# aa2il/pySDR

Hardware: AMD Instinct MI355X
Metric: complex IQ MS/s through 4-RX demod chain (higher is better)
Workload: dtype f32; 1 GPU; C3: 8 MS/s synthetic IQ, 4 RX (USB/CW/NFM/AM), 255-tap prototype 3/500, + 64k-FFT RF PSD on every sample; 2048 chunks x 170666 in HBM; parallelism=stream-sharded x1

## Files before the change

### pysdr_amd/csrc/api.hip

```cpp
#include <dlfcn.h>
#include <rccl/rccl.h>
#include <rocfft/rocfft.h>

#include <cmath>
#include <algorithm>
#include <cstdarg>
#include <map>

#include "common.h"
#include "host_plan.h"
#include "host_res.h"
#include "mixdec_mfma_geom.h"
#include "mixdec_plan.h"
#include "objects_plan.h"

namespace pysdr {

static thread_local char g_err[2048] = "";

void set_last_error(const char* fmt, ...) {
  va_list ap;
  va_start(ap, fmt);
  vsnprintf(g_err, sizeof(g_err), fmt, ap);
  va_end(ap);
// ... 1262 lines not shown
    float pk = 0.f;
    rc = pysdr_fetch(c, r, outs[r].am, outs[r].iq, outs[r].cap, &nout, &cx, nullptr, &pk);
    if (rc) return rc;
    outs[r].n_out = nout;
    outs[r].am_is_complex = cx;
    outs[r].peak_in = pk;
  }
  return PYSDR_OK;
}

int pysdr_quad_mixer(int device, const float* x, float* y, size_t n, uint32_t phase0,
                     uint32_t fword, uint32_t* phase_out) {
  if (!x || !y) return PYSDR_ERR_ARG;
  int rc = use_device(device);
  if (rc) return rc;
  if (phase_out) *phase_out = phase0 + fword * (uint32_t)n;
  if (n == 0) return PYSDR_OK;
  DevBuf<float2> dx, dy;
  PYSDR_HIP_CHECK(dx.alloc(n));
  PYSDR_HIP_CHECK(dy.alloc(n));
  PYSDR_HIP_CHECK(hipMemcpy(dx.get(), x, n * sizeof(float2), hipMemcpyHostToDevice));
  rc = launch_quad_mixer(dx.get(), dy.get(), n, phase0, fword, nullptr);
  if (rc) return rc;
  PYSDR_HIP_CHECK(hipMemcpy(y, dy.get(), n * sizeof(float2), hipMemcpyDeviceToHost));
  return PYSDR_OK;
}

int pysdr_fir_real(int device, const float* xx, const float* h, int ntaps, float* y, size_t n) {
  if (!xx || !h || !y || ntaps < 1) return PYSDR_ERR_ARG;
  if (n == 0) return PYSDR_OK;
  int rc = use_device(device);
  if (rc) return rc;
  const size_t nin = n + (size_t)ntaps - 1;
  DevBuf<float> dx, dh, dy;
  PYSDR_HIP_CHECK(dx.alloc(nin));
  PYSDR_HIP_CHECK(dh.alloc((size_t)ntaps));
  PYSDR_HIP_CHECK(dy.alloc(n));
  PYSDR_HIP_CHECK(hipMemcpy(dx.get(), xx, nin * sizeof(float), hipMemcpyHostToDevice));
  PYSDR_HIP_CHECK(hipMemcpy(dh.get(), h, (size_t)ntaps * sizeof(float), hipMemcpyHostToDevice));
  rc = launch_fir_real(dx.get(), dh.get(), ntaps, dy.get(), (int)n, nullptr);
  if (rc) return rc;
  PYSDR_HIP_CHECK(hipMemcpy(y, dy.get(), n * sizeof(float), hipMemcpyDeviceToHost));
  return PYSDR_OK;
}

static int get_plan(pysdr_spectrum* sp, int batch, rocfft_plan* out) {
  auto it = sp->plans.find(batch);
  if (it != sp->plans.end()) { *out = it->second; return PYSDR_OK; }
  rocfft_plan plan = nullptr;
  size_t len[1] = {(size_t)sp->nfft};
  rocfft_status s = rocfft_plan_create(&plan, rocfft_placement_inplace, rocfft_transform_type_complex_forward,
                                       rocfft_precision_single, 1, len, (size_t)batch, nullptr);
  if (s != rocfft_status_success) { set_last_error("rocfft_plan_create(nfft=%d,batch=%d) = %d", sp->nfft, batch, (int)s); return PYSDR_ERR_FFT; }
  size_t wbs = 0;
  rocfft_plan_get_work_buffer_size(plan, &wbs);
  const hipError_t e = sp->d_fftwork.grow(wbs);
  if (e != hipSuccess) {
    rocfft_plan_destroy(plan);
    set_last_error("rocFFT work buffer of %zu bytes: %s", wbs, hipGetErrorString(e));
    return PYSDR_ERR_HIP;
  }
  if (sp->d_fftwork) rocfft_execution_info_set_work_buffer(sp->info, sp->d_fftwork.get(), sp->d_fftwork.size());
  sp->plans[batch] = plan;
  *out = plan;
  return PYSDR_OK;
}

static int spectrum_alloc(pysdr_spectrum* sp, const float* window) {
  PYSDR_HIP_CHECK(sp->stream.create(hipStreamNonBlocking));
  PYSDR_HIP_CHECK(sp->d_win.alloc((size_t)sp->chunk));
  PYSDR_HIP_CHECK(hipMemcpy(sp->d_win.get(), window, (size_t)sp->chunk * sizeof(float), hipMemcpyHostToDevice));
  PYSDR_HIP_CHECK(sp->d_in.alloc((size_t)sp->chunk));
  PYSDR_HIP_CHECK(sp->d_out.alloc((size_t)sp->nfft));
  PYSDR_HIP_CHECK(sp->ev[0].create());
  PYSDR_HIP_CHECK(sp->ev[1].create());
  return PYSDR_OK;
}

int pysdr_spectrum_create(int device, int chunk_size, int nfft, int max_frames, const float* window,
                          pysdr_spectrum** out) {
  if (!out || !window || chunk_size < 1 || nfft < chunk_size || max_frames < 1) return PYSDR_ERR_ARG;
  int rc = use_device(device);
  if (rc) return rc;
  {
    std::lock_guard<std::mutex> lk(g_rocfft_mu);
    if (g_rocfft_users++ == 0) rocfft_setup();
  }
  pysdr_spectrum* sp = new pysdr_spectrum();
  sp->device = device; sp->chunk = chunk_size; sp->nfft = nfft; sp->max_frames = max_frames;
  sp->tune = SpectrumTuning::from_env();
  {
    hipDeviceProp_t prop;
    if (hipGetDeviceProperties(&prop, device) == hipSuccess && prop.multiProcessorCount > 0) sp->num_cus = prop.multiProcessorCount;
  }
  rc = spectrum_alloc(sp, window);
  if (rc) { failed_in("pysdr_spectrum_create", rc); pysdr_spectrum_destroy(sp); return rc; }
  if (rocfft_execution_info_create(&sp->info) != rocfft_status_success ||
      rocfft_execution_info_set_stream(sp->info, sp->stream.get()) != rocfft_status_success) {
    set_last_error("rocfft_execution_info_create failed");
    pysdr_spectrum_destroy(sp);
    return PYSDR_ERR_FFT;
  }
  *out = sp;
  return PYSDR_OK;
}

void pysdr_spectrum_destroy(pysdr_spectrum* sp) {
  if (!sp) return;
  (void)hipSetDevice(sp->device);
  if (sp->stream) (void)hipStreamSynchronize(sp->stream);
  for (int i = 1; i < pysdr_spectrum::kMaxStreams; ++i) if (sp->xstream[i]) (void)hipStreamSynchronize(sp->xstream[i]);
  for (auto& kv : sp->plans) rocfft_plan_destroy(kv.second);
  if (sp->info) rocfft_execution_info_destroy(sp->info);
  delete sp;
  std::lock_guard<std::mutex> lk(g_rocfft_mu);
  if (--g_rocfft_users == 0) rocfft_cleanup();
}

static int ensure_work(pysdr_spectrum* sp, size_t frames) {
  const size_t n = frames * (size_t)sp->nfft;
  if (sp->d_work.size() >= n) return PYSDR_OK;
  PYSDR_HIP_CHECK(hipStreamSynchronize(sp->stream));
  PYSDR_HIP_CHECK(sp->d_work.grow(n));
  return PYSDR_OK;
}

static int spectrum_run(pysdr_spectrum* sp, const float2* d_x, size_t hop, int nframes, int is_complex,
                        int db, float* d_out) {
  int rc;
  if (is_complex && sp->chunk == 32768 && sp->nfft == 65536 && !sp->tune.force_rocfft) {
    const int group = sp->tune.frames_per_group();
    if (sp->tune.nstreams > 1 && nframes > group) {
      const int ns = sp->tune.nstreams;
      const int part = (group + ns - 1) / ns;
      rc = ensure_work(sp, (size_t)part);
      if (rc) return rc;
      if (sp->xwork_frames < (size_t)part) {
        for (int i = 1; i < ns; ++i) {
          if (!sp->xstream[i]) PYSDR_HIP_CHECK(sp->xstream[i].create(hipStreamNonBlocking));
          if (!sp->ev_join[i]) PYSDR_HIP_CHECK(sp->ev_join[i].create(hipEventDisableTiming));
          PYSDR_HIP_CHECK(hipStreamSynchronize(sp->xstream[i]));
          PYSDR_HIP_CHECK(sp->xwork[i].alloc((size_t)part * sp->nfft));
        }
        sp->xwork_frames = (size_t)part;
      }
      PYSDR_HIP_CHECK(hipEventRecord(sp->ev[0], sp->stream));
      for (int i = 1; i < ns; ++i) PYSDR_HIP_CHECK(hipStreamWaitEvent(sp->xstream[i], sp->ev[0], 0));
      int k = 0;
      for (int f0 = 0; f0 < nframes; f0 += part, ++k) {
        const int nf = (nframes - f0 < part) ? nframes - f0 : part;
        const int w = k % ns;
        rc = launch_psd64k(d_x + (size_t)f0 * hop, hop, nf, sp->d_win.get(), w ? sp->xwork[w].get() : sp->d_work.get(),
                           d_out + (size_t)f0 * sp->nfft, db, w ? sp->xstream[w].get() : sp->stream.get(),
                           psd_form(sp->tune, nf, sp->num_cus));
        if (rc) break;
      }
      for (int i = 1; i < ns; ++i) {
        PYSDR_HIP_CHECK(hipEventRecord(sp->ev_join[i], sp->xstream[i]));
        PYSDR_HIP_CHECK(hipStreamWaitEvent(sp->stream, sp->ev_join[i], 0));
      }
      PYSDR_HIP_CHECK(hipEventRecord(sp->ev[1], sp->stream));
      return rc;
    }
    rc = ensure_work(sp, (size_t)std::min(group, nframes));
    if (rc) return rc;
    PYSDR_HIP_CHECK(hipEventRecord(sp->ev[0], sp->stream));
    for (int f0 = 0; f0 < nframes; f0 += group) {
      const int nf = (nframes - f0 < group) ? nframes - f0 : group;
      rc = launch_psd64k(d_x + (size_t)f0 * hop, hop, nf, sp->d_win.get(), sp->d_work.get(),
                         d_out + (size_t)f0 * sp->nfft, db, sp->stream, psd_form(sp->tune, nf, sp->num_cus));
      if (rc) return rc;
    }
    PYSDR_HIP_CHECK(hipEventRecord(sp->ev[1], sp->stream));
    return PYSDR_OK;
  }
  rocfft_plan plan;
  rc = get_plan(sp, nframes, &plan);
  if (rc) return rc;
  rc = ensure_work(sp, (size_t)nframes);
  if (rc) return rc;
  PYSDR_HIP_CHECK(hipEventRecord(sp->ev[0], sp->stream));
  rc = launch_psd_pre(d_x, hop, nframes, sp->chunk, sp->nfft, sp->d_win.get(), sp->d_work.get(), is_complex, sp->stream);
  if (rc) return rc;
  void* bufs[1] = {sp->d_work.get()};
  rocfft_status s = rocfft_execute(plan, bufs, nullptr, sp->info);
  if (s != rocfft_status_success) { set_last_error("rocfft_execute = %d", (int)s); return PYSDR_ERR_FFT; }
  rc = launch_psd_post(sp->d_work.get(), nframes, sp->nfft, is_complex ? 0 : 1, db, d_out, sp->stream);
  if (rc) return rc;
  PYSDR_HIP_CHECK(hipEventRecord(sp->ev[1], sp->stream));
  return PYSDR_OK;
}

int pysdr_spectrum_frame(pysdr_spectrum* sp, const float* x, int is_complex, int db, float* psd_out,
                         int* n_out) {
  if (!sp || !x || !psd_out) return PYSDR_ERR_ARG;
  int rc = use_device(sp->device);
  if (rc) return rc;
  const size_t bytes = (size_t)sp->chunk * (is_complex ? sizeof(float2) : sizeof(float));
  PYSDR_HIP_CHECK(hipMemcpyAsync(sp->d_in.get(), x, bytes, hipMemcpyHostToDevice, sp->stream));
  rc = spectrum_run(sp, sp->d_in.get(), 0, 1, is_complex, db, sp->d_out.get());
  if (!rc) sp->ran = true;
  if (rc) return rc;
  const int nout = is_complex ? sp->nfft : sp->nfft / 2;
  PYSDR_HIP_CHECK(hipMemcpyAsync(psd_out, sp->d_out.get(), (size_t)nout * sizeof(float), hipMemcpyDeviceToHost, sp->stream));
  PYSDR_HIP_CHECK(hipStreamSynchronize(sp->stream));
  if (n_out) *n_out = nout;
  return PYSDR_OK;
}

int pysdr_spectrum_batch(pysdr_spectrum* sp, const void* d_iq, int nframes, size_t hop, void* d_out) {
  if (!sp || !d_iq || !d_out || nframes < 1 || nframes > sp->max_frames) return PYSDR_ERR_ARG;
  int rc = use_device(sp->device);
  if (rc) return rc;
  rc = spectrum_run(sp, reinterpret_cast<const float2*>(d_iq), hop, nframes, 1, 1, reinterpret_cast<float*>(d_out));
  if (!rc) sp->ran = true;
  return rc;
}

int pysdr_spectrum_get_tuning(pysdr_spectrum* sp, int32_t out[4]) {
  if (!sp || !out) return PYSDR_ERR_ARG;
  out[0] = sp->tune.frames_per_group(); out[1] = sp->tune.force_rocfft ? 1 : 0; out[2] = sp->tune.nstreams; out[3] = sp->tune.packed;
  return PYSDR_OK;
}

int pysdr_spectrum_sync(pysdr_spectrum* sp) {
  if (!sp) return PYSDR_ERR_ARG;
  int rc = use_device(sp->device);
  if (rc) return rc;
  PYSDR_HIP_CHECK(hipStreamSynchronize(sp->stream));
  return PYSDR_OK;
}

int pysdr_spectrum_elapsed_ms(pysdr_spectrum* sp, float* ms) {
  if (!sp || !ms) return PYSDR_ERR_ARG;
  int rc = use_device(sp->device);
  if (rc) return rc;
  PYSDR_HIP_CHECK(hipEventSynchronize(sp->ev[1]));
  PYSDR_HIP_CHECK(hipEventElapsedTime(ms, sp->ev[0], sp->ev[1]));
  return PYSDR_OK;
}

int pysdr_spectrum_order(pysdr_spectrum* sp, pysdr_ctx* c, int direction) {
  if (!sp || !c || direction < 0 || direction > 2 || sp->device != c->cfg.device) return PYSDR_ERR_ARG;
  std::lock_guard<std::recursive_mutex> run_lk(c->run_mu);
  int rc = use_device(sp->device);
  if (rc) return rc;
  if (direction == 2) {
    c->front_wanted = 1;
    if (c->front_marker) {
      PYSDR_HIP_CHECK(hipStreamWaitEvent(sp->stream, c->front_marker, 0));
      return PYSDR_OK;
    }
    direction = 0;
  }
  if (direction == 1 && sp->ran) {
    PYSDR_HIP_CHECK(hipStreamWaitEvent(c->stream, sp->ev[1], 0));
    return PYSDR_OK;
  }
  if (!sp->ev_order) PYSDR_HIP_CHECK(sp->ev_order.create(hipEventDisableTiming));
  if (direction == 0) { rc = flush_tail(c); if (rc) return rc; }
  hipStream_t first = direction == 0 ? c->stream : sp->stream;
  hipStream_t then = direction == 0 ? sp->stream : c->stream;
  PYSDR_HIP_CHECK(hipEventRecord(sp->ev_order, first));
  PYSDR_HIP_CHECK(hipStreamWaitEvent(then, sp->ev_order, 0));
  return PYSDR_OK;
}

int pysdr_dev_alloc(int device, size_t bytes, void** out) {
  if (!out || bytes == 0) return PYSDR_ERR_ARG;
  int rc = use_device(device);
  if (rc) return rc;
  PYSDR_HIP_CHECK(hipMalloc(out, bytes));
  return PYSDR_OK;
}
int pysdr_dev_free(int device, void* p) {
  if (!p) return PYSDR_OK;
  int rc = use_device(device);
  if (rc) return rc;
  PYSDR_HIP_CHECK(hipFree(p));
  return PYSDR_OK;
}
int pysdr_dev_upload(int device, void* dst, const void* src_host, size_t bytes) {
  if (!dst || !src_host) return PYSDR_ERR_ARG;
  int rc = use_device(device);
  if (rc) return rc;
  PYSDR_HIP_CHECK(hipMemcpy(dst, src_host, bytes, hipMemcpyHostToDevice));
  return PYSDR_OK;
}
int pysdr_dev_download(int device, void* dst_host, const void* src, size_t bytes) {
  if (!dst_host || !src) return PYSDR_ERR_ARG;
  int rc = use_device(device);
  if (rc) return rc;
  PYSDR_HIP_CHECK(hipMemcpy(dst_host, src, bytes, hipMemcpyDeviceToHost));
  return PYSDR_OK;
}
int pysdr_dev_copy(int device, void* dst, const void* src, size_t bytes) {
  if (!dst || !src) return PYSDR_ERR_ARG;
  int rc = use_device(device);
  if (rc) return rc;
  PYSDR_HIP_CHECK(hipMemcpy(dst, src, bytes, hipMemcpyDeviceToDevice));
  return PYSDR_OK;
}

void pysdr_ingest_destroy(pysdr_ingest* g) {
  if (!g) return;
  if (g->c) (void)hipSetDevice(g->c->cfg.device);
  if (g->copy_stream) (void)hipStreamSynchronize(g->copy_stream);
  if (g->c && g->c->stream) (void)hipStreamSynchronize(g->c->stream);
  if (g->c && g->counted) { g->c->n_ingest--; g->counted = false; }
  delete g;
}

static int ingest_alloc(pysdr_ingest* g) {
  const int nslots = g->nslots;
  PYSDR_HIP_CHECK(g->copy_stream.create(hipStreamNonBlocking));
  g->h_in.resize(nslots);
  g->ev_copied.resize(nslots);
  g->ev_done.resize(nslots);
  g->h_am.resize((size_t)nslots * PYSDR_MAX_RX);
  g->h_iq.resize((size_t)nslots * PYSDR_MAX_RX);
  g->h_peak.resize(nslots);
  g->n_out.assign(nslots, 0);
  g->in_flight.assign(nslots, 0);
// ... 217 lines not shown
```

### pysdr_amd/csrc/host_plan.h

```cpp
#pragma once

#include <algorithm>
#include <cmath>
#include <cstdlib>
#include <cstring>

#include "common.h"

namespace pysdr {

constexpr double kTwo32 = 4294967296.0;
constexpr double kPllBwHz = 50.0, kPllZeta = 0.7071;
constexpr double kWfmPllBwHz = 30.0;
constexpr int kPllSegMax = 8192;

inline const char* tuning_env(const char* name) {
  const char* on = getenv("PYSDR_TUNING");
  if (!on || atoi(on) <= 0) return nullptr;
  return getenv(name);
}

struct Tuning {
  int tile_bytes = 0, threads = 1024;
  int wgs_per_cu = 1;
  int grid_override = 0;
  int resamp_plain = 0;
  int mfma_enable = 1;
  int dbg_flags = 0, yflush_cap = 0;
  int overlap_env = -1;
  int tail_first = -1;
  bool overlap_prio_set = false;
  int overlap_prio = 0;
  double am_taus = 16.0, am_taus_exact = 5.0;
  int am_coarse_sweeps = 4, am_kmax = 2048, am_tmin = 512;
  int am_seeded = 1, am_wseed = 0;
  int am_direct = 1;
  int am_phase_on_2 = 1;
  double wfm_taus = 20.0, wfm_taus_fast = 13.0, wfm_taus_exact = 4.0;
  int wfm_coarse_sweeps = 3, wfm_kmax = 1536, wfm_tmin = 2048;
  double wfm_taus_hi = 0.0, wfm_taus_mid = 0.0;
  int wfm_tail_cap = 0;
  int wfm_exact_cap = 5;
  int wfm_seeded = 1, wfm_wseed = 0;

  static Tuning from_env() {
    Tuning t;
    { const char* e = tuning_env("PYSDR_MIXDEC_WGS"); if (e && atoi(e) > 0) t.wgs_per_cu = atoi(e); }
    { const char* e = tuning_env("PYSDR_MIXDEC_YFLUSH"); if (e && atoi(e) > 0) t.yflush_cap = atoi(e); }
    { const char* e = tuning_env("PYSDR_AM_PLL");
      if (e && *e) {
        double a = 0, tx = 0; int cs = 0, km = 0, tm = 0;
        const int nf = sscanf(e, "%lf,%lf,%d,%d,%d", &a, &tx, &cs, &km, &tm);
        if (nf >= 1 && a > 0) t.am_taus = a;
        if (nf >= 2 && tx >= 0) t.am_taus_exact = tx;
        if (nf >= 3 && cs >= 0) t.am_coarse_sweeps = std::min(cs, 8);
        if (nf >= 4 && km > 0) t.am_kmax = std::min(km, kPllSegMax);
        if (nf >= 5 && tm >= 64) t.am_tmin = (tm + 63) & ~63;
      } }
    { const char* e = tuning_env("PYSDR_AM_SEED");
      if (e && *e) { int on = 1, ws = 0; const int nf = sscanf(e, "%d,%d", &on, &ws); if (nf >= 1) t.am_seeded = on ? 1 : 0; if (nf >= 2 && ws >= 0) t.am_wseed = ws; } }
    { const char* e = tuning_env("PYSDR_AM_DIRECT"); if (e && *e) t.am_direct = atoi(e) ? 1 : 0; }
    { const char* e = tuning_env("PYSDR_AM_PHASE_STREAM"); if (e && *e) t.am_phase_on_2 = atoi(e) ? 1 : 0; }
    { const char* e = tuning_env("PYSDR_MIXDEC_MFMA"); if (e && *e) t.mfma_enable = atoi(e) ? 1 : 0; }
    { const char* e = tuning_env("PYSDR_WFM_SEED");
      if (e && *e) { int on = 1, ws = 0; const int nf = sscanf(e, "%d,%d", &on, &ws); if (nf >= 1) t.wfm_seeded = on ? 1 : 0; if (nf >= 2 && ws >= 0) t.wfm_wseed = ws; } }
    { const char* e = tuning_env("PYSDR_OVERLAP_ORDER"); if (e && *e) t.tail_first = atoi(e); }
    { const char* e = tuning_env("PYSDR_OVERLAP"); if (e && *e) t.overlap_env = std::max(0, std::min(2, atoi(e))); }
    { const char* e = tuning_env("PYSDR_OVERLAP_PRIO"); if (e && *e) { t.overlap_prio_set = true; t.overlap_prio = atoi(e); } }
    { const char* e = tuning_env("PYSDR_RESAMP_PLAIN"); if (e && *e) t.resamp_plain = atoi(e); }
    { const char* e = tuning_env("PYSDR_MIXDEC_GRID"); if (e && atoi(e) > 0) t.grid_override = atoi(e); }
    { const char* e = tuning_env("PYSDR_WFM_PLL");
      if (e && *e) {
        double a = t.wfm_taus, b = t.wfm_taus_fast, x = t.wfm_taus_exact;
        int sw = t.wfm_coarse_sweeps, km = t.wfm_kmax, tm = t.wfm_tmin, xc = t.wfm_exact_cap;
        double th = t.wfm_taus_hi, tmid = t.wfm_taus_mid;
        int tc = t.wfm_tail_cap;
        const int got = sscanf(e, "%lf,%lf,%lf,%d,%d,%d,%d,%lf,%lf,%d", &a, &b, &x, &sw, &km, &tm, &xc, &th, &tmid, &tc);
        if (got >= 10 && tc >= 0) t.wfm_tail_cap = tc;
        if (got >= 9 && th >= 0 && tmid >= 0) { t.wfm_taus_hi = th; t.wfm_taus_mid = tmid; }
        if (got >= 7 && xc >= 0) t.wfm_exact_cap = xc;
        if (got >= 1 && a > 0) t.wfm_taus = a;
        if (got >= 2 && b >= 0) t.wfm_taus_fast = b;
        if (got >= 3 && x > 0) t.wfm_taus_exact = x;
        if (got >= 4 && sw >= 0) t.wfm_coarse_sweeps = sw;
        if (got >= 5 && km >= 1) t.wfm_kmax = std::min(km, kPllSegMax);
        if (got >= 6 && tm >= 64) t.wfm_tmin = tm;
      } }
#ifdef PYSDR_DIAG
    { const char* e = getenv("PYSDR_DEBUG_FLAGS"); t.dbg_flags = e ? atoi(e) : 0; }
#endif
    return t;
  }
};

constexpr int kPsdColsMaxG = 4096;
struct SpectrumTuning {
  bool force_rocfft = false;
  int group = 0;
  int packed = 1;
  static constexpr int kMaxStreams = 4;
  int nstreams = 2;
  int cols_g = -1;
  int frames_per_group() const { return group > 0 ? group : (packed ? 480 : 448); }

  static SpectrumTuning from_env() {
    SpectrumTuning t;
    t.force_rocfft = tuning_env("PYSDR_PSD_ROCFFT") != nullptr;
    { const char* e = tuning_env("PYSDR_PSD_GROUP"); if (e && atoi(e) > 0) t.group = atoi(e); }
    { const char* e = tuning_env("PYSDR_PSD_PACKED"); if (e && *e) t.packed = atoi(e) ? 1 : 0; }
    { const char* e = tuning_env("PYSDR_PSD_STREAMS"); if (e && atoi(e) >= 1 && atoi(e) <= kMaxStreams) t.nstreams = atoi(e); }
    { const char* e = tuning_env("PYSDR_PSD_PATH");
      if (e && !strcmp(e, "unit")) t.cols_g = 0;
      else if (e && !strncmp(e, "loop:", 5) && atoi(e + 5) > 0) t.cols_g = std::min(atoi(e + 5), kPsdColsMaxG); }
    return t;
  }
};

constexpr int kPsdColBlocks = 16, kPsdColsWgPerCu = 4;
inline int psd_cols_max_g(int num_cus) { return std::max(1, std::min(kPsdColsMaxG, num_cus * kPsdColsWgPerCu / kPsdColBlocks)); }
inline int plan_psd_cols(int nframes, int num_cus, int forced) {
  if (nframes < 1) return 1;
  if (forced > 0) return std::min(forced, nframes);
  const int gmax = psd_cols_max_g(num_cus);
  const int rounds = (nframes + gmax - 1) / gmax;
  return (nframes + rounds - 1) / rounds;
}
inline int psd_form(const SpectrumTuning& t, int nframes, int num_cus) {
  if (!t.packed) return 0;
  return t.cols_g == 0 ? 1 : 1 + plan_psd_cols(nframes, num_cus, t.cols_g);
}

inline int round_up64(int v) { return (v + 63) & ~63; }
inline double pll_tau(double fs, double bw_hz) { return fs / (kPllZeta * 2.0 * M_PI * bw_hz); }
inline int pll_warmup(double taus, double tau) { return round_up64((int)std::ceil(taus * tau)); }

inline PllPlan plan_pll(int n, double tau, double taus, double taus_fast, int t_min, int k_max, uint32_t* seg) {
  PllPlan p;
  p.W = pll_warmup(taus, tau);
  p.Wfast = taus_fast > 0 ? pll_warmup(taus_fast, tau) : 0;
  p.Wexact = 0;
  p.Wc_hi = p.Wc_mid = 0;
  p.tail_cap = 0;
  p.coarse_sweeps = 0;
  p.exact_cap = 0;
  p.seeded = 0;
  p.Wseed = 0;
  p.direct = 0;
  if (n < 3 * p.W || k_max <= 1) {
    p.K = 1;
    p.T = round_up64(std::max(n, 64));
  } else {
    p.T = std::max(t_min, round_up64((n + k_max - 1) / k_max));
    p.K = (n + p.T - 1) / p.T;
  }
  p.seg = seg;
  p.lin = seg + (size_t)PYSDR_MAX_RX * kPllSegMax * 4;
  return p;
}

inline PllPlan plan_am_pll(const Tuning& t, int n_out, double fs_out, int pll_kmax, uint32_t* seg) {
  const double tau = pll_tau(fs_out, kPllBwHz);
  PllPlan p = plan_pll(n_out, tau, t.am_taus, 0.0, t.am_tmin, pll_kmax > 0 ? std::min(pll_kmax, t.am_kmax) : t.am_kmax, seg);
  if (t.am_coarse_sweeps > 0 && p.K > 1) {
    p.Wexact = pll_warmup(t.am_taus_exact, tau);
    p.coarse_sweeps = t.am_coarse_sweeps;
  }
  p.seeded = (t.am_seeded && p.K > 1) ? 1 : 0;
  p.direct = t.am_direct;
  p.Wseed = std::min(round_up64(std::max(0, t.am_wseed)), std::max(0, p.W - 64));
  return p;
}

inline PllPlan plan_wfm_pll(const Tuning& t, int n1, double fs1, int pll_kmax, uint32_t* seg) {
  const double tau = pll_tau(fs1, kWfmPllBwHz);
  PllPlan p = plan_pll(n1, tau, t.wfm_taus, t.wfm_taus_fast, t.wfm_tmin, pll_kmax > 0 ? std::min(pll_kmax, t.wfm_kmax) : t.wfm_kmax, seg);
  p.exact_cap = t.wfm_exact_cap;
  p.tail_cap = t.wfm_tail_cap;
  p.seeded = (t.wfm_seeded && p.K > 1) ? 1 : 0;
  p.Wseed = round_up64(std::max(0, t.wfm_wseed));
  if (t.wfm_coarse_sweeps > 0 && p.K > 1) {
    p.Wexact = pll_warmup(t.wfm_taus_exact, tau);
    p.coarse_sweeps = t.wfm_coarse_sweeps;
    if (t.wfm_taus_hi > 0 || t.wfm_taus_mid > 0) {
      p.Wc_hi = pll_warmup(t.wfm_taus_hi, tau);
      p.Wc_mid = pll_warmup(t.wfm_taus_mid, tau);
    }
  }
  return p;
}

inline WfmArgs wfm_args(int nrx, int n1, double fs1) {
  WfmArgs w;
  memset(&w, 0, sizeof(w));
  w.nrx = nrx; w.n1 = n1;
  w.scale = (float)(fs1 / (2.0 * M_PI * 75e3));
  const double wn = 2.0 * M_PI * kWfmPllBwHz / fs1;
  w.kp = (float)(2.0 * kPllZeta * wn);
  w.ki = (float)(wn * wn);
  w.norm = (float)(2.0 / 0.1);
  w.rad2word = (float)(kTwo32 / (2.0 * M_PI));
  w.fword0 = pysdr_freq_word(19000.0, fs1, nullptr);
  return w;
}

}
```

### pysdr_amd/csrc/psdfft.hip

```cpp
#include <algorithm>

#include "common.h"
#include "psd_cols_geom.h"

namespace pysdr {

namespace {

constexpr int kN = 65536, kM = 32768;

__device__ __forceinline__ float2 cmul(float2 a, float2 b) {
  return make_float2(fmaf(a.x, b.x, -a.y * b.y), fmaf(a.x, b.y, a.y * b.x));
}
__device__ __forceinline__ float2 cadd(float2 a, float2 b) { return make_float2(a.x + b.x, a.y + b.y); }
__device__ __forceinline__ float2 csub(float2 a, float2 b) { return make_float2(a.x - b.x, a.y - b.y); }
__device__ __forceinline__ float2 expmpi(float t) {
  const float rev = 0.5f * t;
  return make_float2(__builtin_amdgcn_cosf(rev), -__builtin_amdgcn_sinf(rev));
}

typedef float v2f_t __attribute__((ext_vector_type(2)));
#define PYSDR_AS1 __attribute__((address_space(1)))
__device__ __forceinline__ float2 ldg2(const float2* p) {
  const v2f_t v = *(const PYSDR_AS1 v2f_t*)p;
  return make_float2(v.x, v.y);
}
__device__ __forceinline__ void stg2(float2* p, float2 v) {
  const v2f_t w = {v.x, v.y};
  *(PYSDR_AS1 v2f_t*)p = w;
}
__device__ __forceinline__ float2 ldg2_stream(const float2* p) {
  const v2f_t v = __builtin_nontemporal_load((const PYSDR_AS1 v2f_t*)p);
  return make_float2(v.x, v.y);
}
__device__ __forceinline__ void stg1_stream(float* p, float v) {
  __builtin_nontemporal_store(v, (PYSDR_AS1 float*)p);
}
__device__ __forceinline__ float ldg1(const float* p) {
  return *(const PYSDR_AS1 float*)p;
}
__device__ __forceinline__ void stg1(float* p, float v) {
  *(PYSDR_AS1 float*)p = v;
}

__device__ __forceinline__ void dft4(float2& a, float2& b, float2& c, float2& d) {
  const float2 s0 = cadd(a, c), s1 = csub(a, c), s2 = cadd(b, d), s3 = csub(b, d);
  a = cadd(s0, s2);
  c = csub(s0, s2);
  b = make_float2(s1.x + s3.y, s1.y - s3.x);
  d = make_float2(s1.x - s3.y, s1.y + s3.x);
}

__device__ __forceinline__ void dft16(float2 (&v)[16]) {
  const float c1 = 0.92387953251128674f, s1 = 0.38268343236508977f;
  const float h = 0.70710678118654752f;
#pragma unroll
  for (int n0 = 0; n0 < 4; ++n0) dft4(v[n0], v[n0 + 4], v[n0 + 8], v[n0 + 12]);
  v[5] = cmul(v[5], make_float2(c1, -s1));
  v[9] = cmul(v[9], make_float2(h, -h));
  v[13] = cmul(v[13], make_float2(s1, -c1));
  v[6] = cmul(v[6], make_float2(h, -h));
  v[10] = make_float2(v[10].y, -v[10].x);
  v[14] = cmul(v[14], make_float2(-h, -h));
  v[7] = cmul(v[7], make_float2(s1, -c1));
  v[11] = cmul(v[11], make_float2(-h, -h));
  v[15] = cmul(v[15], make_float2(-c1, s1));
#pragma unroll
  for (int k1 = 0; k1 < 4; ++k1) dft4(v[4 * k1], v[4 * k1 + 1], v[4 * k1 + 2], v[4 * k1 + 3]);
#pragma unroll
  for (int i = 0; i < 4; ++i)
#pragma unroll
    for (int j = i + 1; j < 4; ++j) {
      const float2 t = v[4 * i + j];
      v[4 * i + j] = v[4 * j + i];
      v[4 * j + i] = t;
    }
}

__device__ __forceinline__ void twiddle_pow0(float2 (&v)[16], float2 w, float2 w0) {
  const float2 w2 = cmul(w, w), w4 = cmul(w2, w2), w8 = cmul(w4, w4);
  const float2 b0 = w0, b4 = cmul(w0, w4), b8 = cmul(w0, w8), b12 = cmul(b4, w8);
  const float2 w3 = cmul(w2, w);
  v[0] = cmul(v[0], b0); v[1] = cmul(v[1], cmul(b0, w)); v[2] = cmul(v[2], cmul(b0, w2)); v[3] = cmul(v[3], cmul(b0, w3));
  v[4] = cmul(v[4], b4); v[5] = cmul(v[5], cmul(b4, w)); v[6] = cmul(v[6], cmul(b4, w2)); v[7] = cmul(v[7], cmul(b4, w3));
  v[8] = cmul(v[8], b8); v[9] = cmul(v[9], cmul(b8, w)); v[10] = cmul(v[10], cmul(b8, w2)); v[11] = cmul(v[11], cmul(b8, w3));
  v[12] = cmul(v[12], b12); v[13] = cmul(v[13], cmul(b12, w)); v[14] = cmul(v[14], cmul(b12, w2)); v[15] = cmul(v[15], cmul(b12, w3));
}
constexpr int kTwRow = 17;
__device__ __forceinline__ void tw256_build(float2* tw, int tid) {
  if (tid < 256) tw[kTwRow * (tid >> 4) + (tid & 15)] = expmpi((float)((tid >> 4) * (tid & 15)) * (1.0f / 128.0f));
}
__device__ __forceinline__ void twiddle_tab(float2 (&v)[16], const float2* tw, int i) {
  const float2* r = tw + kTwRow * i;
#pragma unroll
  for (int k = 1; k < 16; ++k) v[k] = cmul(v[k], r[k]);
}

constexpr int kColsPerWg = 16;
constexpr int kColLds = 16 * 272;

__device__ __forceinline__ void cols_unit(const float2* __restrict__ xf, const float* __restrict__ win,
                                          float2* __restrict__ yf, int cb, int tid, float2* lds,
                                          const float2* tw) {
  const int b = tid & 15, hi = tid >> 4;
  const int bb = cb * kColsPerWg + b;
  {
    const int a0 = hi;
    float2 u[16];
#pragma unroll
    for (int a1 = 0; a1 < 8; ++a1) {
      const int n = 256 * (a0 + 16 * a1) + bb;
      const float2 s = ldg2_stream(xf + n);
      const float g = ldg1(win + n);
      u[a1] = make_float2(s.x * g, s.y * g);
    }
#pragma unroll
    for (int a1 = 8; a1 < 16; ++a1) u[a1] = make_float2(0.f, 0.f);
    dft16(u);
    __syncthreads();
    twiddle_tab(u, tw, a0);
    float2* p = lds + 16 * a0 + b;
#pragma unroll
    for (int p1 = 0; p1 < 16; ++p1) p[272 * p1] = u[p1];
  }
  __syncthreads();
  {
    const int p1 = hi;
    const float2* p = lds + 272 * p1 + b;
    float2 v[16];
#pragma unroll
    for (int a0 = 0; a0 < 16; ++a0) v[a0] = p[16 * a0];
    dft16(v);
    twiddle_pow0(v, expmpi((float)(16 * bb) * (1.0f / 32768.0f)),
                 expmpi((float)(bb * p1) * (1.0f / 32768.0f)));
    float2* o = yf + (size_t)cb * 4096 + p1 * 16 + b;
#pragma unroll
    for (int p0 = 0; p0 < 16; ++p0) stg2(o + p0 * 256, v[p0]);
  }
}

__global__ __launch_bounds__(256) void psd_cols_kernel(const float2* __restrict__ x, size_t hop,
                                                       const float* __restrict__ win,
                                                       float2* __restrict__ work) {
  __shared__ __attribute__((aligned(16))) float2 lds[kColLds];
  __shared__ __attribute__((aligned(16))) float2 tw[16 * kTwRow];
  const int f = blockIdx.y;
  tw256_build(tw, threadIdx.x);
  cols_unit(x + (size_t)f * hop, win, work + (size_t)f * kN, blockIdx.x, threadIdx.x, lds, tw);
}

constexpr int kRowsPerWg = 32;
constexpr int kRowLds = 16 * 544;

template <bool kBypassL1>
__device__ __forceinline__ float2 load_work(const float2* p) {
  if (kBypassL1) {
// ... 111 lines not shown
      ol[p0 * 256] = (unsigned short)pk_perm(c, a, 0x0c0c0400u);
    }
  }
}

__global__ __launch_bounds__(256) void psd_cols_pk_unit_kernel(const float2* __restrict__ x, size_t hop,
                                                               const float* __restrict__ win, char* __restrict__ work) {
  __shared__ __attribute__((aligned(16))) float2 lds[kColLds];
  __shared__ __attribute__((aligned(16))) float2 tw[16 * kTwRow];
  __shared__ float red[4];
  const int f = blockIdx.y;
  tw256_build(tw, threadIdx.x);
  cols_unit_pk(x + (size_t)f * hop, win, work + (size_t)f * kN * sizeof(float2), blockIdx.x, threadIdx.x, lds, tw, red);
}


__device__ __forceinline__ void cols_prefetch(v2f_t (&nx)[8], unsigned voff, const float2* xf) {
  const PYSDR_AS1 char* base = (const PYSDR_AS1 char*)xf;
#pragma unroll
  for (int a1 = 0; a1 < 8; ++a1)
    asm volatile("global_load_dwordx2 %0, %1, %2 nt" : "+v"(nx[a1]) : "v"(voff), "s"(base + 32768 * a1));
}
__device__ __forceinline__ void cols_prefetch_wait(v2f_t (&nx)[8]) {
  asm volatile("s_waitcnt vmcnt(0)"
               : "+v"(nx[0]), "+v"(nx[1]), "+v"(nx[2]), "+v"(nx[3]), "+v"(nx[4]), "+v"(nx[5]), "+v"(nx[6]), "+v"(nx[7]));
}

__global__ __launch_bounds__(256, 4) void psd_cols_pk_kernel(const float2* __restrict__ x, size_t hop,
                                                             const float* __restrict__ win, char* __restrict__ work,
                                                             int nframes) {
  __shared__ __attribute__((aligned(16))) float2 lds[kColLds];
  __shared__ __attribute__((aligned(16))) float2 tw[16 * kTwRow];
  __shared__ float red[4];
  const int tid = threadIdx.x, cb = blockIdx.x;
  const int b = tid & 15, hi = tid >> 4;
  const int bb = cb * kColsPerWg + b;
  PsdColsWalk fr((int)blockIdx.y, (int)gridDim.y, nframes);
  const unsigned voff = (unsigned)(256 * hi + bb) * (unsigned)sizeof(float2);
  v2f_t nx[8] = {};
  cols_prefetch(nx, voff, x + (size_t)fr.f * hop);
  tw256_build(tw, tid);
  float g[8];
#pragma unroll
  for (int a1 = 0; a1 < 8; ++a1) g[a1] = ldg1(win + 256 * (hi + 16 * a1) + bb);
  float2 t[16];
  {
    const float2 w = expmpi((float)(16 * bb) * (1.0f / 32768.0f)), w0 = expmpi((float)(bb * hi) * (1.0f / 32768.0f));
    const float2 w2 = cmul(w, w), w4 = cmul(w2, w2), w8 = cmul(w4, w4);
    const float2 b0 = w0, b4 = cmul(w0, w4), b8 = cmul(w0, w8), b12 = cmul(b4, w8);
    const float2 w3 = cmul(w2, w);
    t[0] = b0; t[1] = cmul(b0, w); t[2] = cmul(b0, w2); t[3] = cmul(b0, w3);
    t[4] = b4; t[5] = cmul(b4, w); t[6] = cmul(b4, w2); t[7] = cmul(b4, w3);
    t[8] = b8; t[9] = cmul(b8, w); t[10] = cmul(b8, w2); t[11] = cmul(b8, w3);
    t[12] = b12; t[13] = cmul(b12, w); t[14] = cmul(b12, w2); t[15] = cmul(b12, w3);
  }
  float2* const p1w = lds + 16 * hi + b;
  const float2* const p2r = lds + 272 * hi + b;
  const size_t oidx = (size_t)cb * 4096 + hi * 16 + b;
  cols_prefetch_wait(nx);
  __syncthreads();
  for (;;) {
    float2 u[16];
#pragma unroll
    for (int a1 = 0; a1 < 8; ++a1) {
      u[a1] = make_float2(nx[a1].x * g[a1], nx[a1].y * g[a1]);
      asm volatile("" : "+v"(u[a1].x), "+v"(u[a1].y));
    }
#pragma unroll
    for (int a1 = 8; a1 < 16; ++a1) u[a1] = make_float2(0.f, 0.f);
    if (fr.has_next()) cols_prefetch(nx, voff, x + (size_t)fr.fn * hop);
    dft16(u);
    twiddle_tab(u, tw, hi);
#pragma unroll
    for (int p1 = 0; p1 < 16; ++p1) p1w[272 * p1] = u[p1];
    __syncthreads();
    float2 v[16];
#pragma unroll
    for (int a0 = 0; a0 < 16; ++a0) v[a0] = p2r[16 * a0];
    dft16(v);
#pragma unroll
    for (int k = 0; k < 16; ++k) v[k] = cmul(v[k], t[k]);
    float m = 0.f;
#pragma unroll
    for (int p0 = 0; p0 < 16; ++p0) m = fmaxf(fmaxf(m, fabsf(v[p0].x)), fabsf(v[p0].y));
#pragma unroll
    for (int o = 32; o > 0; o >>= 1) m = fmaxf(m, __shfl_xor(m, o));
    red[tid >> 6] = m;
    __syncthreads();
    m = fmaxf(fmaxf(red[0], red[1]), fmaxf(red[2], red[3]));
    const bool live = m >= 1.0e-20f;
    const float sc = live ? __fdiv_rn(8388600.0f, m) : 0.0f;
    char* const wf = work + (size_t)fr.f * kN * sizeof(float2);
    cols_prefetch_wait(nx);
    if ((tid & 63) == 0)
      *(PYSDR_AS1 float*)(wf + kPkScaleOff + 4 * (4 * cb + (tid >> 6))) = live ? __fdiv_rn(m, 8388600.0f) * (1.0f / 256.0f) : 0.f;
    PYSDR_AS1 unsigned* oh = (PYSDR_AS1 unsigned*)wf + oidx;
    PYSDR_AS1 unsigned short* ol = (PYSDR_AS1 unsigned short*)(wf + kPkLoOff) + oidx;
#pragma unroll
    for (int p0 = 0; p0 < 16; ++p0) {
      const unsigned a = (unsigned)__float2int_rn(v[p0].x * sc), c = (unsigned)__float2int_rn(v[p0].y * sc);
      oh[p0 * 256] = pk_perm(c, a, 0x06050201u);
      ol[p0 * 256] = (unsigned short)pk_perm(c, a, 0x0c0c0400u);
    }
    if (!fr.has_next()) break;
    fr.advance();
  }
}

__device__ __forceinline__ void rows_unit_pk(const char* __restrict__ wf, float* __restrict__ of, int rb, int db,
                                             int tid, float2* lds, const float2* tw) {
  {
    const int c0 = tid & 15, pl = tid >> 4;
    const size_t idx = (size_t)(rb * kRowsPerWg + pl) * 16 + c0;
    const PYSDR_AS1 unsigned* sh = (const PYSDR_AS1 unsigned*)wf + idx;
    const PYSDR_AS1 unsigned short* sl = (const PYSDR_AS1 unsigned short*)(wf + kPkLoOff) + idx;
    const PYSDR_AS1 float* ss = (const PYSDR_AS1 float*)(wf + kPkScaleOff);
    unsigned h[16], l[16];
#pragma unroll
    for (int c1 = 0; c1 < 16; ++c1) { h[c1] = sh[4096 * c1]; l[c1] = sl[4096 * c1]; }
    float2 u[16];
#pragma unroll
    for (int c1 = 0; c1 < 16; ++c1) {
      const float inv = ss[4 * c1 + ((tid >> 6) & 3)];
      const int xr = (int)pk_perm(l[c1], h[c1], 0x0100040cu);
      const int xi = (int)pk_perm(l[c1], h[c1], 0x0302050cu);
      u[c1] = make_float2((float)xr * inv, (float)xi * inv);
    }
    dft16(u);
    __syncthreads();
    twiddle_tab(u, tw, c0);
    float2* p = lds + 17 * pl + c0;
#pragma unroll
    for (int q1 = 0; q1 < 16; ++q1) p[544 * q1] = u[q1];
  }
  __syncthreads();
  {
    const int pl = tid & 31, q1 = tid >> 5;
    const float2* p = lds + 544 * q1 + 17 * pl;
    float2 v[16];
#pragma unroll
    for (int c0 = 0; c0 < 16; ++c0) v[c0] = p[c0];
    dft16(v);
    const int kb = rb * kRowsPerWg + pl + 256 * q1;
#pragma unroll
    for (int q0 = 0; q0 < 16; ++q0) {
      const int k = kb + 4096 * q0;
      float pw = v[q0].x * v[q0].x + v[q0].y * v[q0].y;
      if (db) pw = 3.0102999566398120f * __builtin_amdgcn_logf(pw + 1.0e-30f);
      stg1_stream(of + ((k + kM) & (kN - 1)), pw);
    }
  }
}

__global__ __launch_bounds__(512) void psd_rows_pk_kernel(const char* __restrict__ work, float* __restrict__ out, int db) {
  __shared__ __attribute__((aligned(16))) float2 lds[kRowLds];
  __shared__ __attribute__((aligned(16))) float2 tw[16 * kTwRow];
  const int f = blockIdx.y;
  tw256_build(tw, threadIdx.x);
  rows_unit_pk(work + (size_t)f * kN * sizeof(float2), out + (size_t)f * kN, blockIdx.x, db, threadIdx.x, lds, tw);
}

}

int launch_psd64k(const float2* x, size_t hop, int nframes, const float* win, float2* work,
                  float* out, int db, hipStream_t st, int form) {
  if (form >= 1) {
    if (form > 1) {
      const int rows = std::min(form - 1, nframes);
      hipLaunchKernelGGL(psd_cols_pk_kernel, dim3(256 / kColsPerWg, rows), dim3(256), 0, st, x, hop, win, (char*)work, nframes);
    } else {
      hipLaunchKernelGGL(psd_cols_pk_unit_kernel, dim3(256 / kColsPerWg, nframes), dim3(256), 0, st, x, hop, win, (char*)work);
    }
    PYSDR_HIP_CHECK(hipGetLastError());
    hipLaunchKernelGGL(psd_rows_pk_kernel, dim3(256 / kRowsPerWg, nframes), dim3(512), 0, st, (const char*)work, out, db);
    PYSDR_HIP_CHECK(hipGetLastError());
    return PYSDR_OK;
  }
  hipLaunchKernelGGL(psd_cols_kernel, dim3(256 / kColsPerWg, nframes), dim3(256), 0, st, x, hop, win,
                     work);
  PYSDR_HIP_CHECK(hipGetLastError());
  hipLaunchKernelGGL(psd_rows_kernel, dim3(256 / kRowsPerWg, nframes), dim3(512), 0, st, work, out, db);
  PYSDR_HIP_CHECK(hipGetLastError());
  return PYSDR_OK;
}

}
```

Baseline: 119,700 MS/s.

## Add persistent frame-looping PSD rows kernel with software-prefetched next frame

Adds a persistent version of the packed PSD rows kernel. It launches a grid sized to the CU count (about two workgroups per CU over 8 row blocks) and loops over frames. Each iteration prefetches the next frame's packed high/low/scale data into registers with inline global and scalar loads while the current frame's DFT, twiddle and LDS transpose run, and the twiddle table is built once per workgroup. The goal is to hide load latency and cut per-frame launch and setup costs, at the price of higher register pressure from the double-buffered registers, hand-written asm waits that must be correct, and less parallelism when there are few frames.

```diff
diff --git a/pysdr_amd/csrc/api.hip b/pysdr_amd/csrc/api.hip
--- a/pysdr_amd/csrc/api.hip
+++ b/pysdr_amd/csrc/api.hip
@@ -1438,7 +1438,7 @@
         const int w = k % ns;
         rc = launch_psd64k(d_x + (size_t)f0 * hop, hop, nf, sp->d_win.get(), w ? sp->xwork[w].get() : sp->d_work.get(),
                            d_out + (size_t)f0 * sp->nfft, db, w ? sp->xstream[w].get() : sp->stream.get(),
-                           psd_form(sp->tune, nf, sp->num_cus));
+                           psd_launch_form(sp->tune, nf, sp->num_cus));
         if (rc) break;
       }
       for (int i = 1; i < ns; ++i) {
@@ -1454,7 +1454,7 @@
     for (int f0 = 0; f0 < nframes; f0 += group) {
       const int nf = (nframes - f0 < group) ? nframes - f0 : group;
       rc = launch_psd64k(d_x + (size_t)f0 * hop, hop, nf, sp->d_win.get(), sp->d_work.get(),
-                         d_out + (size_t)f0 * sp->nfft, db, sp->stream, psd_form(sp->tune, nf, sp->num_cus));
+                         d_out + (size_t)f0 * sp->nfft, db, sp->stream, psd_launch_form(sp->tune, nf, sp->num_cus));
       if (rc) return rc;
     }
     PYSDR_HIP_CHECK(hipEventRecord(sp->ev[1], sp->stream));
diff --git a/pysdr_amd/csrc/host_plan.h b/pysdr_amd/csrc/host_plan.h
--- a/pysdr_amd/csrc/host_plan.h
+++ b/pysdr_amd/csrc/host_plan.h
@@ -94,13 +94,14 @@
 };
 
 constexpr int kPsdColsMaxG = 4096;
+constexpr int kPsdRowsMaxR = 4096;
 struct SpectrumTuning {
   bool force_rocfft = false;
   int group = 0;
   int packed = 1;
   static constexpr int kMaxStreams = 4;
   int nstreams = 2;
-  int cols_g = -1;
+  int cols_g = -1, rows_r = -1;
   int frames_per_group() const { return group > 0 ? group : (packed ? 480 : 448); }
 
   static SpectrumTuning from_env() {
@@ -110,8 +111,20 @@
     { const char* e = tuning_env("PYSDR_PSD_PACKED"); if (e && *e) t.packed = atoi(e) ? 1 : 0; }
     { const char* e = tuning_env("PYSDR_PSD_STREAMS"); if (e && atoi(e) >= 1 && atoi(e) <= kMaxStreams) t.nstreams = atoi(e); }
     { const char* e = tuning_env("PYSDR_PSD_PATH");
-      if (e && !strcmp(e, "unit")) t.cols_g = 0;
-      else if (e && !strncmp(e, "loop:", 5) && atoi(e + 5) > 0) t.cols_g = std::min(atoi(e + 5), kPsdColsMaxG); }
+      bool rows_given = false;
+      while (e && *e) {
+        const char* end = strchr(e, ',');
+        const size_t len = end ? (size_t)(end - e) : strlen(e);
+        const bool rows = len >= 5 && !strncmp(e, "rows=", 5);
+        const char* p = rows ? e + 5 : e;
+        const size_t plen = rows ? len - 5 : len;
+        int v = -1;
+        if (plen == 4 && !strncmp(p, "unit", 4)) v = 0;
+        else if (plen > 5 && !strncmp(p, "loop:", 5) && atoi(p + 5) > 0) v = std::min(atoi(p + 5), rows ? kPsdRowsMaxR : kPsdColsMaxG);
+        if (rows) { t.rows_r = v; rows_given = true; } else t.cols_g = v;
+        e = end ? end + 1 : nullptr;
+      }
+      if (!rows_given && t.cols_g == 0) t.rows_r = 0; }
     return t;
   }
 };
@@ -128,6 +141,25 @@
 inline int psd_form(const SpectrumTuning& t, int nframes, int num_cus) {
   if (!t.packed) return 0;
   return t.cols_g == 0 ? 1 : 1 + plan_psd_cols(nframes, num_cus, t.cols_g);
+}
+
+constexpr int kPsdRowBlocks = 8, kPsdRowsWgPerCu = 2;
+inline int psd_rows_max_r(int num_cus) { return std::max(1, std::min(kPsdRowsMaxR, num_cus * kPsdRowsWgPerCu / kPsdRowBlocks)); }
+inline int plan_psd_rows(int nframes, int num_cus, int forced) {
+  if (nframes < 1) return 1;
+  if (forced > 0) return std::min(forced, nframes);
+  const int rmax = psd_rows_max_r(num_cus);
+  const int rounds = (nframes + rmax - 1) / rmax;
+  return (nframes + rounds - 1) / rounds;
+}
+inline int psd_rows_form(const SpectrumTuning& t, int nframes, int num_cus) {
+  if (!t.packed || t.rows_r == 0) return 0;
+  return plan_psd_rows(nframes, num_cus, t.rows_r);
+}
+constexpr int kPsdRowsFormShift = 16;
+static_assert(kPsdColsMaxG + 1 < (1 << kPsdRowsFormShift) && kPsdRowsMaxR < (1 << (31 - kPsdRowsFormShift)), "the two forms share an int");
+inline int psd_launch_form(const SpectrumTuning& t, int nframes, int num_cus) {
+  return psd_form(t, nframes, num_cus) | (psd_rows_form(t, nframes, num_cus) << kPsdRowsFormShift);
 }
 
 inline int round_up64(int v) { return (v + 63) & ~63; }
diff --git a/pysdr_amd/csrc/psd_rows_geom.h b/pysdr_amd/csrc/psd_rows_geom.h
--- /dev/null
+++ b/pysdr_amd/csrc/psd_rows_geom.h
@@ -0,0 +1,18 @@
+#pragma once
+
+#if defined(__HIPCC__)
+#define PYSDR_PSD_ROWS_HD __device__ __forceinline__
+#else
+#define PYSDR_PSD_ROWS_HD inline
+#endif
+
+namespace pysdr {
+
+struct PsdRowsWalk {
+  int f, fn, R, nframes;
+  PYSDR_PSD_ROWS_HD PsdRowsWalk(int r, int R_, int nframes_) : f(r), fn(r + R_), R(R_), nframes(nframes_) {}
+  PYSDR_PSD_ROWS_HD bool has_next() const { return fn < nframes; }
+  PYSDR_PSD_ROWS_HD void advance() { f = fn; fn += R; }
+};
+
+}
diff --git a/pysdr_amd/csrc/psdfft.hip b/pysdr_amd/csrc/psdfft.hip
--- a/pysdr_amd/csrc/psdfft.hip
+++ b/pysdr_amd/csrc/psdfft.hip
@@ -2,6 +2,7 @@
 
 #include "common.h"
 #include "psd_cols_geom.h"
+#include "psd_rows_geom.h"
 
 namespace pysdr {
 
@@ -419,7 +420,7 @@
   }
 }
 
-__global__ __launch_bounds__(512) void psd_rows_pk_kernel(const char* __restrict__ work, float* __restrict__ out, int db) {
+__global__ __launch_bounds__(512) void psd_rows_pk_unit_kernel(const char* __restrict__ work, float* __restrict__ out, int db) {
   __shared__ __attribute__((aligned(16))) float2 lds[kRowLds];
   __shared__ __attribute__((aligned(16))) float2 tw[16 * kTwRow];
   const int f = blockIdx.y;
@@ -427,19 +428,114 @@
   rows_unit_pk(work + (size_t)f * kN * sizeof(float2), out + (size_t)f * kN, blockIdx.x, db, threadIdx.x, lds, tw);
 }
 
+
+#define PYSDR_ROWS_SLOAD(c1, off) asm volatile("s_load_dword %0, %1, " #off : "+s"(ns[c1]) : "s"(sbase))
+__device__ __forceinline__ void rows_prefetch(unsigned (&nh)[16], unsigned (&nl)[16], float (&ns)[16], unsigned voh, unsigned vol,
+                                              const char* wf, int wave4) {
+  const PYSDR_AS1 char* base = (const PYSDR_AS1 char*)wf;
+#pragma unroll
+  for (int c1 = 0; c1 < 16; ++c1)
+    asm volatile("global_load_dword %0, %1, %2" : "+v"(nh[c1]) : "v"(voh), "s"(base + 16384 * c1));
+#pragma unroll
+  for (int c1 = 0; c1 < 16; ++c1)
+    asm volatile("global_load_ushort %0, %1, %2" : "+v"(nl[c1]) : "v"(vol), "s"(base + kPkLoOff + 8192 * c1));
+  const PYSDR_AS1 char* sbase = base + kPkScaleOff + wave4;
+  PYSDR_ROWS_SLOAD(0, 0x00); PYSDR_ROWS_SLOAD(1, 0x10); PYSDR_ROWS_SLOAD(2, 0x20); PYSDR_ROWS_SLOAD(3, 0x30);
+  PYSDR_ROWS_SLOAD(4, 0x40); PYSDR_ROWS_SLOAD(5, 0x50); PYSDR_ROWS_SLOAD(6, 0x60); PYSDR_ROWS_SLOAD(7, 0x70);
+  PYSDR_ROWS_SLOAD(8, 0x80); PYSDR_ROWS_SLOAD(9, 0x90); PYSDR_ROWS_SLOAD(10, 0xa0); PYSDR_ROWS_SLOAD(11, 0xb0);
+  PYSDR_ROWS_SLOAD(12, 0xc0); PYSDR_ROWS_SLOAD(13, 0xd0); PYSDR_ROWS_SLOAD(14, 0xe0); PYSDR_ROWS_SLOAD(15, 0xf0);
+}
+#undef PYSDR_ROWS_SLOAD
+__device__ __forceinline__ void rows_prefetch_wait(unsigned (&nh)[16], unsigned (&nl)[16], float (&ns)[16]) {
+  asm volatile("s_waitcnt vmcnt(0) lgkmcnt(0)"
+               : "+v"(nh[0]), "+v"(nh[1]), "+v"(nh[2]), "+v"(nh[3]), "+v"(nh[4]), "+v"(nh[5]), "+v"(nh[6]), "+v"(nh[7]),
+                 "+v"(nh[8]), "+v"(nh[9]), "+v"(nh[10]), "+v"(nh[11]), "+v"(nh[12]), "+v"(nh[13]), "+v"(nh[14]), "+v"(nh[15]));
+  asm volatile(""
+               : "+v"(nl[0]), "+v"(nl[1]), "+v"(nl[2]), "+v"(nl[3]), "+v"(nl[4]), "+v"(nl[5]), "+v"(nl[6]), "+v"(nl[7]),
+                 "+v"(nl[8]), "+v"(nl[9]), "+v"(nl[10]), "+v"(nl[11]), "+v"(nl[12]), "+v"(nl[13]), "+v"(nl[14]), "+v"(nl[15]));
+  asm volatile(""
+               : "+s"(ns[0]), "+s"(ns[1]), "+s"(ns[2]), "+s"(ns[3]), "+s"(ns[4]), "+s"(ns[5]), "+s"(ns[6]), "+s"(ns[7]),
+                 "+s"(ns[8]), "+s"(ns[9]), "+s"(ns[10]), "+s"(ns[11]), "+s"(ns[12]), "+s"(ns[13]), "+s"(ns[14]), "+s"(ns[15]));
+}
+
+__global__ __launch_bounds__(512, 4) void psd_rows_pk_kernel(const char* __restrict__ work, float* __restrict__ out, int db,
+                                                             int nframes) {
+  __shared__ __attribute__((aligned(16))) float2 lds[kRowLds];
+  __shared__ __attribute__((aligned(16))) float2 tw[16 * kTwRow];
+  const int tid = threadIdx.x, rb = blockIdx.x;
+  PsdRowsWalk fr((int)blockIdx.y, (int)gridDim.y, nframes);
+  const unsigned idx = 512u * (unsigned)rb + (unsigned)tid;
+  const unsigned voh = idx * 4u, vol = idx * 2u;
+  const int wave4 = 4 * __builtin_amdgcn_readfirstlane((tid >> 6) & 3);
+  unsigned nh[16] = {}, nl[16] = {};
+  float ns[16] = {};
+  rows_prefetch(nh, nl, ns, voh, vol, work + (size_t)fr.f * kN * sizeof(float2), wave4);
+  tw256_build(tw, tid);
+  const int c0 = tid & 15;
+  float2* const p1w = lds + 17 * (tid >> 4) + c0;
+  const int pl = tid & 31, q1 = tid >> 5;
+  const float2* const p2r = lds + 544 * q1 + 17 * pl;
+  const unsigned kbo = (unsigned)(rb * kRowsPerWg + pl + 256 * q1) * (unsigned)sizeof(float);
+  rows_prefetch_wait(nh, nl, ns);
+  __syncthreads();
+  for (;;) {
+    float2 u[16];
+#pragma unroll
+    for (int c1 = 0; c1 < 16; ++c1) {
+      const float inv = ns[c1];
+      const int xr = (int)pk_perm(nl[c1], nh[c1], 0x0100040cu);
+      const int xi = (int)pk_perm(nl[c1], nh[c1], 0x0302050cu);
+      u[c1] = make_float2((float)xr * inv, (float)xi * inv);
+      asm volatile("" : "+v"(u[c1].x), "+v"(u[c1].y));
+    }
+    if (fr.has_next()) rows_prefetch(nh, nl, ns, voh, vol, work + (size_t)fr.fn * kN * sizeof(float2), wave4);
+    dft16(u);
+    twiddle_tab(u, tw, c0);
+#pragma unroll
+    for (int k = 0; k < 16; ++k) p1w[544 * k] = u[k];
+    __syncthreads();
+    float2 v[16];
+#pragma unroll
+    for (int k = 0; k < 16; ++k) v[k] = p2r[k];
+    __syncthreads();
+    dft16(v);
+    float pw[16];
+#pragma unroll
+    for (int q0 = 0; q0 < 16; ++q0) {
+      pw[q0] = v[q0].x * v[q0].x + v[q0].y * v[q0].y;
+      if (db) pw[q0] = 3.0102999566398120f * __builtin_amdgcn_logf(pw[q0] + 1.0e-30f);
+    }
+    rows_prefetch_wait(nh, nl, ns);
+    PYSDR_AS1 char* const o = (PYSDR_AS1 char*)(out + (size_t)fr.f * kN);
+#pragma unroll
+    for (int q0 = 0; q0 < 16; ++q0) {
+      PYSDR_AS1 char* oq = o + 16384 * ((q0 + 8) & 15);
+      asm("" : "+s"(oq));
+      __builtin_nontemporal_store(pw[q0], (PYSDR_AS1 float*)(oq + kbo));
+    }
+    if (!fr.has_next()) break;
+    fr.advance();
+  }
+}
+
 }
 
 int launch_psd64k(const float2* x, size_t hop, int nframes, const float* win, float2* work,
                   float* out, int db, hipStream_t st, int form) {
-  if (form >= 1) {
-    if (form > 1) {
-      const int rows = std::min(form - 1, nframes);
+  const int cform = form & 0xffff, rform = form >> 16;
+  if (cform >= 1) {
+    if (cform > 1) {
+      const int rows = std::min(cform - 1, nframes);
       hipLaunchKernelGGL(psd_cols_pk_kernel, dim3(256 / kColsPerWg, rows), dim3(256), 0, st, x, hop, win, (char*)work, nframes);
     } else {
       hipLaunchKernelGGL(psd_cols_pk_unit_kernel, dim3(256 / kColsPerWg, nframes), dim3(256), 0, st, x, hop, win, (char*)work);
     }
     PYSDR_HIP_CHECK(hipGetLastError());
-    hipLaunchKernelGGL(psd_rows_pk_kernel, dim3(256 / kRowsPerWg, nframes), dim3(512), 0, st, (const char*)work, out, db);
+    if (rform > 0) {
+      hipLaunchKernelGGL(psd_rows_pk_kernel, dim3(256 / kRowsPerWg, std::min(rform, nframes)), dim3(512), 0, st, (const char*)work, out, db, nframes);
+    } else {
+      hipLaunchKernelGGL(psd_rows_pk_unit_kernel, dim3(256 / kRowsPerWg, nframes), dim3(512), 0, st, (const char*)work, out, db);
+    }
     PYSDR_HIP_CHECK(hipGetLastError());
     return PYSDR_OK;
   }
```

Measured after the change: 125,800 MS/s, median of 6. 5.1% higher.
